# rossumur/espflix

Measured on NVIDIA H100. Metric: 352x192 MPEG-1 frames/sec (decoded YUV bit-exact vs reference), higher is better.
Workload: dtype int32/u8

## Files before the change

espflix_b200/csrc/ef_decode.cu:

```cuda
#include "ef_common.cuh"
#include "ef_coef_step.cuh"

namespace {

constexpr int kParseThreads = EF_K1A_THREADS;
constexpr int kParseCtasPerSm = EF_K1A_CTAS;
constexpr int kHdrBatch = EF_K1A_HDR_BATCH;
constexpr int kReconWarps = EF_K1B_WARPS;
constexpr int kReconCtasPerSm = EF_K1B_CTAS;

constexpr int kDenseStride = 72;
constexpr int kDenseWords = 6 * kDenseStride;
constexpr int kDenseBytes = kDenseWords * 4;
constexpr int kStageBytes = 4 * EF_TILE;
constexpr int kWarpBytes = 2 * (kDenseBytes + kStageBytes) + 16;
constexpr int kReconQzBytes = EF_K1B_DEQUANT ? 128 * 4 : 0;

struct SharedTables {
    uint16_t dct[26 * 32];
    uint16_t mba[8 * 32];
    uint16_t mv[7 * 32];
    uint16_t cbp[512];
    uint8_t ptype[64];
    uint8_t qdef[128];
    uint16_t zp[64];
    uint32_t qz[128];
};
constexpr int kTableBytes = (sizeof(SharedTables) + 15) & ~15;
constexpr int kLutBits = EF_K1A_LUT_BITS;
constexpr int kLutSize = 1 << kLutBits;
constexpr int kLutBytes = kLutBits > 0 ? 2 * kLutSize * (int)sizeof(uint2) : 0;

#if EF_K1A_ES16
constexpr int kRingStride = kParseThreads * 16;
constexpr int kRingBytes = 4 * kRingStride;
#else
constexpr int kRingStride = kParseThreads * 4;
constexpr int kRingBytes = 8 * kRingStride;
#endif
constexpr int kFlushUnroll = EF_K1A_FLUSH_UNROLL;
constexpr int kStage = EF_K1A_STAGE;
constexpr int kStageRow = EF_K1A_ES16 ? ((kStage * 4 + 16 + 15) & ~15) : (kStage + 1) * 4;
constexpr int kStageBytesA = kStage > 0 ? kParseThreads * kStageRow : 0;

struct BitReader {
    const uint32_t* words;
    uint32_t rp;
    uint32_t sring;
    uint32_t hi, lo;
#if EF_K1A_RING_AHEAD || EF_K1A_ES16
    uint32_t nx;
#endif
    int pos;

#if EF_K1A_ES16
    __device__ __forceinline__ void copy_chunk(uint32_t cidx)
    {
        asm volatile("cp.async.cg.shared.global [%0], [%1], 16;" ::"r"(sring + (cidx & 3u) * kRingStride), "l"((const uint4*)words + cidx) : "memory");
        asm volatile("cp.async.commit_group;" ::: "memory");
    }
    __device__ __forceinline__ void init(const uint8_t* blob, uint64_t byte_off)
    {
        words = (const uint32_t*)blob;
        const uint32_t w0 = (uint32_t)(byte_off >> 2);
        pos = (int)(byte_off & 3) * 8;
        asm volatile("cp.async.wait_all;" ::: "memory");
        rp = w0 + 2;
        const uint32_t c0 = (rp + 1) >> 2;
#pragma unroll
        for (int k = 0; k < 4; k++) copy_chunk(c0 + k);
        hi = __byte_perm(__ldg(words + w0), 0, 0x0123); lo = __byte_perm(__ldg(words + w0 + 1), 0, 0x0123);
        nx = __ldg(words + w0 + 2);
    }
    __device__ __forceinline__ uint32_t peek() const { return __funnelshift_l(lo, hi, pos); }
    __device__ __forceinline__ void skip(int n)
    {
// ... 32 lines not shown
    {
        pos += n;
        if (pos >= 32) {
            pos -= 32; hi = lo;
#if EF_K1A_RING_AHEAD
            lo = __byte_perm(nx, 0, 0x0123);
            asm volatile("cp.async.wait_group 5;" ::: "memory");
            asm volatile("ld.shared.u32 %0, [%1];" : "=r"(nx) : "r"(sring + ((rp + 1) & 7u) * kRingStride) : "memory");
            copy_in(rp + 7);
#else
            asm volatile("cp.async.wait_group 6;" ::: "memory");
            uint32_t raw;
            asm volatile("ld.shared.u32 %0, [%1];" : "=r"(raw) : "r"(sring + (rp & 7u) * kRingStride) : "memory");
            lo = __byte_perm(raw, 0, 0x0123);
            copy_in(rp + 7);
#endif
#if EF_K1A_PF_L2
            if ((rp & 7u) == 0) asm volatile("prefetch.global.L2 [%0];" ::"l"(words + rp + 32));
#endif
            rp++;
        }
    }
#endif
    __device__ __forceinline__ uint32_t get(int n)
    {
        uint32_t v = peek() >> (32 - n);
        skip(n);
        return v;
    }
};

struct SliceState {
    BitReader br;
    uint32_t* wptr;
    uint32_t slot_base;
    uint32_t seqi;
    const uint32_t* qzp;
    const uint32_t* qz;
    int mbw, mbh;
    int mb_x, mb_y;
    int first;
    int ptype, full_pel, r_size;
    int qscale;
    int dc_y, dc_cr, dc_cb;
    int mv_h, mv_v;
};

__device__ __forceinline__ int motion_component(uint32_t w, int& used, const uint16_t* mvtab, int m, int r_size, bool& bad)
{
    const uint32_t bits = w << used;
    int lz = __clz(bits);
    if (lz > 6) { bad = true; return m; }
    uint32_t e = mvtab[lz * 32 + ((bits << (lz + 1)) >> 27)];
    int len = e & 15;
    if (!len) { bad = true; return m; }
    int code = (int)(e >> 4) - 16;
    used += len;
    int d = code;
    if (code != 0 && r_size != 0) {
        d = ((abs(code) - 1) << r_size) + (int)((w << used) >> (32 - r_size)) + 1;
        used += r_size;
        if (code < 0) d = -d;
    }
    int scale = 1 << r_size;
    m += d;
    if (m > (scale << 4) - 1) m -= scale << 5;
    else if (m < -(scale << 4)) m += scale << 5;
// ... 7 lines not shown
    int b3 = v[2] + v[6];
    int b4 = v[5] - v[3];
    int t1 = v[1] + v[7];
    int t2 = v[3] + v[5];
    int b6 = v[1] - v[7];
    int b7 = t1 + t2;
    int m0 = kFinal ? v[0] + 128 : v[0];
    int x4 = ((b6 * 473 - b4 * 196 + 128) >> 8) - b7;
    int x0 = x4 - (((t1 - t2) * 362 + 128) >> 8);
    int x1 = m0 - b1;
    int x2 = (((v[2] - v[6]) * 362 + 128) >> 8) - b3;
    int x3 = m0 + b1;
    int y3 = x1 + x2, y4 = x3 + b3, y5 = x1 - x2, y6 = x3 - b3;
    int y7 = -x0 - ((b4 * 473 + b6 * 196 + 128) >> 8);
    v[0] = b7 + y4; v[1] = x4 + y3; v[2] = y5 - x0; v[3] = y6 - y7;
    v[4] = y6 + y7; v[5] = x0 + y5; v[6] = y3 - x4; v[7] = y4 - b7;
}

__device__ __forceinline__ uint32_t pin4(uint32_t pred, int r0, int r1, int r2, int r3)
{
#if EF_K1B_PIN16
    const uint32_t s01 = __viaddmin_s16x2_relu(__byte_perm(pred, 0, 0x4140), __byte_perm((uint32_t)r0, (uint32_t)r1, 0x6521), 0x00F800F8u);
    const uint32_t s23 = __viaddmin_s16x2_relu(__byte_perm(pred, 0, 0x4342), __byte_perm((uint32_t)r2, (uint32_t)r3, 0x6521), 0x00F800F8u);
    return __byte_perm(s01, s23, 0x6420);
#else
    const int p0 = __viaddmin_s32_relu((int)__byte_perm(pred, 0, 0x4404), r0, 0xF8FF);
    const int p1 = __viaddmin_s32_relu((int)__byte_perm(pred, 0, 0x4414), r1, 0xF8FF);
    const int p2 = __viaddmin_s32_relu((int)__byte_perm(pred, 0, 0x4424), r2, 0xF8FF);
    const int p3 = __viaddmin_s32_relu((int)__byte_perm(pred, 0, 0x4434), r3, 0xF8FF);
    return __byte_perm(__byte_perm(p0, p1, 0x0051), __byte_perm(p2, p3, 0x0051), 0x5410);
#endif
}

__device__ __forceinline__ uint32_t avg2x4(uint32_t a, uint32_t b) { return (a | b) - (((a ^ b) >> 1) & 0x7F7F7F7Fu); }

__device__ __forceinline__ uint32_t avg4x4(uint32_t a, uint32_t b, uint32_t c, uint32_t d)
{
    const uint32_t m = 0x00FF00FFu;
    uint32_t e = (a & m) + (b & m) + (c & m) + (d & m) + 0x00020002u;
    uint32_t o = ((a >> 8) & m) + ((b >> 8) & m) + ((c >> 8) & m) + ((d >> 8) & m) + 0x00020002u;
    return ((e >> 2) & m) | (((o >> 2) & m) << 8);
}

struct PredWords { uint32_t a0, a1, a2, b0, b1, b2; };

__device__ __forceinline__ uint32_t smem_u32(const void* p) { return (uint32_t)__cvta_generic_to_shared(p); }
__device__ __forceinline__ void mbar_init(uint64_t* bar, int count)
{
    asm volatile("mbarrier.init.shared::cta.b64 [%0], %1;" ::"r"(smem_u32(bar)), "r"(count));
    asm volatile("fence.mbarrier_init.release.cluster;" ::: "memory");
}
__device__ __forceinline__ void mbar_expect_tx(uint32_t sbar, uint32_t bytes)
{
    asm volatile("mbarrier.arrive.expect_tx.shared::cta.b64 _, [%0], %1;" ::"r"(sbar), "r"(bytes) : "memory");
}
__device__ __forceinline__ void bulk_tiles(uint32_t sdst, const uint8_t* gsrc, uint32_t bytes, uint32_t sbar)
{
    asm volatile("cp.async.bulk.shared::cluster.global.mbarrier::complete_tx::bytes [%0], [%1], %2, [%3];"
                 ::"r"(sdst), "l"(gsrc), "r"(bytes), "r"(sbar) : "memory");
}
__device__ __forceinline__ void mbar_wait(uint32_t sbar, uint32_t parity)
{
    uint32_t ok;
    do {
        asm volatile("{ .reg .pred p; mbarrier.try_wait.parity.shared::cta.b64 p, [%1], %2; selp.u32 %0, 1, 0, p; }"
                     : "=r"(ok) : "r"(sbar), "r"(parity) : "memory");
    } while (!ok);
}

template <bool kLuma>
__device__ __forceinline__ void pred_words_staged(const uint8_t* st, int plane, int x, int y, int tx0, int ty0, bool yh, PredWords& w)
{
    constexpr int TS = kLuma ? 16 : 8, SH = kLuma ? 4 : 3;
    const int xa = x & ~3, xi = xa & (TS - 1), yi = y & (TS - 1);
    const int o0 = ((y >> SH) - ty0) * (2 * EF_TILE) + ((xa >> SH) - tx0) * EF_TILE + (kLuma ? 0 : 256 + plane * 64) + yi * TS + xi;
    const int o1 = o0 + (xi + 4 < TS ? 4 : EF_TILE + 4 - TS);
    const int xj = (xi + 4) & (TS - 1);
    int o2 = o1 + (xj + 4 < TS ? 4 : EF_TILE + 4 - TS);
    if (((xa + 8) >> SH) - tx0 > 1) o2 = o1;
    w.a0 = *(const uint32_t*)(st + o0); w.a1 = *(const uint32_t*)(st + o1); w.a2 = *(const uint32_t*)(st + o2);
    if (yh) {
        const int d = yi == TS - 1 ? 2 * EF_TILE - (TS - 1) * TS : TS;
        w.b0 = *(const uint32_t*)(st + o0 + d); w.b1 = *(const uint32_t*)(st + o1 + d); w.b2 = *(const uint32_t*)(st + o2 + d);
    }
}

template <bool kLuma>
__device__ __forceinline__ void pred_words_clamped(const uint8_t* ref, int plane, int x, int y, bool yh, PredWords& w)
{
    constexpr int W = kLuma ? EF_W : EF_W / 2, H = kLuma ? EF_H : EF_H / 2, TS = kLuma ? 16 : 8, SH = kLuma ? 4 : 3;
    const int plane_off = kLuma ? 0 : 256 + plane * 64;
#pragma unroll
    for (int r = 0; r < 2; r++) {
        if (r == 1 && !yh) break;
        const int yy = max(0, min(H - 1, y + r));
        const int xa = max(0, min(W - 4, x & ~3)), xb = min(W - 4, xa + 4), xc = min(W - 4, xa + 8);
        const int rowbase = (yy >> SH) * EF_MBW_MAX * EF_TILE + plane_off + (yy & (TS - 1)) * TS;
        const uint32_t v0 = *(const uint32_t*)(ref + rowbase + (xa >> SH) * EF_TILE + (xa & (TS - 1)));
        const uint32_t v1 = *(const uint32_t*)(ref + rowbase + (xb >> SH) * EF_TILE + (xb & (TS - 1)));
        const uint32_t v2 = *(const uint32_t*)(ref + rowbase + (xc >> SH) * EF_TILE + (xc & (TS - 1)));
        if (r == 0) { w.a0 = v0; w.a1 = v1; w.a2 = v2; } else { w.b0 = v0; w.b1 = v1; w.b2 = v2; }
    }
}

__device__ __forceinline__ void pred_finish(const PredWords& w, int x, int xh, int yh, uint32_t& o0, uint32_t& o1)
{
    const int sh = (x & 3) * 8;
    const uint32_t p0 = __funnelshift_r(w.a0, w.a1, sh), p1 = __funnelshift_r(w.a1, w.a2, sh);
    if (xh) {
        const uint32_t q0 = __funnelshift_rc(w.a0, w.a1, sh + 8), q1 = __funnelshift_rc(w.a1, w.a2, sh + 8);
        if (yh) {
            o0 = avg4x4(p0, q0, __funnelshift_r(w.b0, w.b1, sh), __funnelshift_rc(w.b0, w.b1, sh + 8));
            o1 = avg4x4(p1, q1, __funnelshift_r(w.b1, w.b2, sh), __funnelshift_rc(w.b1, w.b2, sh + 8));
        } else {
            o0 = avg2x4(p0, q0);
            o1 = avg2x4(p1, q1);
        }
    } else if (yh) {
        o0 = avg2x4(p0, __funnelshift_r(w.b0, w.b1, sh));
        o1 = avg2x4(p1, __funnelshift_r(w.b1, w.b2, sh));
    } else {
        o0 = p0; o1 = p1;
    }
}

__device__ __forceinline__ bool parse_header(SliceState& s, const SharedTables& T, int& cbp_out, int& intra_out, uint32_t& skip_out, uint32_t& mv_out)
{
    BitReader& br = s.br;
    uint32_t bits = br.peek();
    if ((bits >> 9) == 0) return false;

    int increment = 0, used;
    uint32_t w;
    for (;;) {
        w = br.peek();
        int lz = __clz(w);
        if (lz > 7) return false;
        uint32_t e = T.mba[lz * 32 + ((w << (lz + 1)) >> 27)];
        int len = e & 15, val = (int)(e >> 4);
        if (!len) return false;
        if (val >= 34) {
            br.skip(len);
            if (val == 35) increment += 33;
            continue;
        }
        increment += val;
        used = len;
        break;
    }
    int skip_before = 0;
    if (s.first) { s.first = 0; increment = 1; }
    else if (increment > 1) { s.dc_y = s.dc_cr = s.dc_cb = 128; s.mv_h = s.mv_v = 0; skip_before = increment - 1; }
    s.mb_x += increment;
// ... 70 lines not shown
        if (delta & (1 << (dc_size - 1))) dc += delta;
        else dc += (int)((0xFFFFFFFFu << dc_size) | (uint32_t)(delta + 1));
        if (blk < 4) s.dc_y = dc; else if (blk == 4) s.dc_cr = dc; else s.dc_cb = dc;
    }
    br.skip(used + dc_size);
    return dc;
}

}

__global__ void __launch_bounds__(kParseThreads, kParseCtasPerSm)
ef_parse_kernel(const __grid_constant__ EfDev D, int pic0, int n_pics)
{
    extern __shared__ __align__(16) uint8_t smem[];
    SharedTables& T = *(SharedTables*)smem;
    const uint2* lut = (const uint2*)(smem + kTableBytes);
    {
        const uint32_t* src = (const uint32_t*)D.tables;
        uint32_t* dst = (uint32_t*)smem;
        for (int i = threadIdx.x; i < (int)(sizeof(SharedTables) / 4); i += blockDim.x) dst[i] = src[i];
        const uint4* lsrc = (const uint4*)D.tables->lut2;
        uint4* ldst = (uint4*)(smem + kTableBytes);
        for (int i = threadIdx.x; i < kLutBytes / 16; i += blockDim.x) ldst[i] = lsrc[i];
    }
    __syncthreads();
    const int lane = threadIdx.x & 31;

    uint32_t total = 0;
    for (int p = pic0; p < pic0 + n_pics; p++) total += D.pic_total[p];
    const EfWork* work = D.work + D.pic_base[pic0];
    const uint32_t n_slots = (uint32_t)D.n_streams * (EF_MBW_MAX * EF_MBH_MAX);

    SliceState s;
    s.first = 0; s.wptr = nullptr; s.slot_base = 0; s.qz = nullptr; s.mbw = 0; s.mb_x = s.mb_y = 0;
    s.br.sring = smem_u32(smem + kTableBytes + kLutBytes) + threadIdx.x * (EF_K1A_ES16 ? 16 : 4);
    const uint32_t sstage_warp = smem_u32(smem + kTableBytes + kLutBytes + kRingBytes) + (threadIdx.x & ~31u) * kStageRow;
#if EF_K1A_ES16
    const uint32_t sstage_bias = smem_u32(smem + kTableBytes + kLutBytes + kRingBytes) - (kStageRow / 16) * smem_u32(smem + kTableBytes + kLutBytes);
#define EF_SSTAGE (s.br.sring * (kStageRow / 16) + sstage_bias)
#else
    const uint32_t sstage = sstage_warp + lane * kStageRow;
#define EF_SSTAGE sstage
#endif
    bool active = false, exhausted = false, busy = false;
    uint32_t info_acc = 0, cnt = 0, skipw = 0, mvw = 0, slot = 0;
    uint32_t blk24 = 0, blkbit = 0;
    int cbp_rem = 0, n = 0, intra = 0, ctx = 0;
    auto start_block = [&]() {
        const int blk = __ffs(cbp_rem) - 1;
#if EF_K1B_DEQUANT
        blk24 = ((uint32_t)blk << 27) | ((uint32_t)s.qscale << 16);
#else
        blk24 = (uint32_t)blk << 24;
#endif
        blkbit = 0x100u << blk;
        cbp_rem &= cbp_rem - 1;
        n = 0; ctx = 1;
        if (intra) { D.mb_rec[slot].dc[blk] = parse_dc(s, blk); n = 1; ctx = 0; }
    };
    auto put_entry = [&](uint32_t ent) {
#if EF_PROBE_NOSTORE
        if (ent == 0x12345678u) s.wptr[cnt] = ent;
#else
        if (kStage > 0 && cnt < (uint32_t)kStage) asm volatile("st.shared.u32 [%0], %1;" ::"r"(EF_SSTAGE + cnt * 4), "r"(ent) : "memory");
        else s.wptr[cnt] = ent;
#endif
        cnt++;
    };
    const uint32_t first_round = gridDim.x * blockDim.x;
    bool first_fill = true;

    for (;;) {
        if (kStage > 0) {
            __syncwarp();
            const uint64_t li_mine = (uint64_t)(s.wptr - D.coef);
            if (kStage <= 32 && kHdrBatch == 32) {
                const uint32_t c_mine = (!busy && (info_acc & 1u)) ? min(cnt, (uint32_t)kStage) : 0u;
                if (__any_sync(0xFFFFFFFFu, c_mine != 0)) {
                    const uint32_t srow = sstage_warp + lane * 4;
#pragma unroll (kFlushUnroll)
                    for (int src = 0; src < 32; src++) {
                        const uint32_t c = __shfl_sync(0xFFFFFFFFu, c_mine, src);
                        const uint64_t lb = (uint64_t)__shfl_sync(0xFFFFFFFFu, (uint32_t)li_mine, src) | ((uint64_t)__shfl_sync(0xFFFFFFFFu, (uint32_t)(li_mine >> 32), src) << 32);
                        if (lane < c) {
                            uint32_t v;
                            asm volatile("ld.shared.u32 %0, [%1];" : "=r"(v) : "r"(srow + (uint32_t)src * kStageRow) : "memory");
                            D.coef[lb + lane] = v;
                        }
                    }
                }
            } else {
                unsigned owed = __ballot_sync(0xFFFFFFFFu, !busy && (info_acc & 1u) && cnt != 0);
                while (owed) {
                    const int src = __ffs(owed) - 1;
                    owed &= owed - 1;
                    const uint32_t c = min(__shfl_sync(0xFFFFFFFFu, cnt, src), (uint32_t)kStage);
                    const uint64_t lb = (uint64_t)__shfl_sync(0xFFFFFFFFu, (uint32_t)li_mine, src) | ((uint64_t)__shfl_sync(0xFFFFFFFFu, (uint32_t)(li_mine >> 32), src) << 32);
                    for (uint32_t j = lane; j < c; j += 32) {
                        uint32_t v;
                        asm volatile("ld.shared.u32 %0, [%1];" : "=r"(v) : "r"(sstage_warp + (uint32_t)src * kStageRow + j * 4) : "memory");
                        D.coef[lb + j] = v;
                    }
                }
            }
            __syncwarp();
        }
        if (!busy && (info_acc & 1u)) {
            const uint64_t li = (uint64_t)(s.wptr - D.coef);
            *(uint4*)(D.mb_rec + slot) = make_uint4(cnt | (skipw << 16), mvw, (uint32_t)li, (uint32_t)(li >> 32));
            s.wptr += cnt;
#if EF_K1B_DEQUANT
            if (s.qz) { info_acc |= 1u << 26; D.mb_rec[slot].pad[0] = s.seqi; }
#endif
            D.mb_info[slot] = info_acc | ((uint32_t)s.mbw << 20) | ((s.slot_base >> 31) << 25);
            info_acc = 0;
        }
        do {
            unsigned need = __ballot_sync(0xFFFFFFFFu, !active && !exhausted);
            if (need) {
                uint32_t base;
                if (first_fill) {
                    base = (blockIdx.x * blockDim.x + threadIdx.x) & ~31u;
                    first_fill = false;
                } else {
                    base = 0;
                    int leader = __ffs(need) - 1;
                    if (lane == leader) base = first_round + atomicAdd(D.parse_cursor, (uint32_t)__popc(need));
                    base = __shfl_sync(0xFFFFFFFFu, base, leader);
                }
                if (!active && !exhausted) {
                    uint32_t idx = base + (uint32_t)__popc(need & ((1u << lane) - 1));
                    if (idx >= total) exhausted = true;
                    else {
                        const EfWork w = work[idx];
                        const int code = w.info & 255;
                        s.ptype = (w.info >> 8) & 7; s.full_pel = (w.info >> 11) & 1; s.r_size = (w.info >> 12) & 7;
                        const EfSeq* seq = D.seq + (size_t)w.stream * (D.max_seq + 1) + (w.info >> 16);
                        s.mbw = min((int)seq->mb_width, EF_MBW_MAX);
                        s.mbh = min((int)seq->mb_height, EF_MBH_MAX);
                        s.qz = seq->custom ? (const uint32_t*)seq->qz : nullptr;
                        s.seqi = w.info >> 16;
                        s.qzp = s.qz ? s.qz : T.qz;
                        const uint64_t byte_off = D.es_off[w.stream] + w.es_off;
                        s.slot_base = (w.pic - (uint32_t)pic0) * n_slots + w.stream * (uint32_t)(EF_MBW_MAX * EF_MBH_MAX);
                        s.slot_base |= ((D.base_pics[w.stream] + w.pic + 1u) & 1u) << 31;
                        s.wptr = D.coef + 3 * byte_off;
                        s.br.init(D.es, byte_off);
                        s.mb_y = code - 2; s.mb_x = s.mbw - 1;
                        s.first = 1;
                        s.dc_y = s.dc_cr = s.dc_cb = 128; s.mv_h = s.mv_v = 0;
                        active = code >= 1 && code <= s.mbh && s.mbw > 0 && seq->valid;
                        if (active) {
                            s.qscale = (int)s.br.get(5);
                            while (s.br.get(1)) s.br.skip(8);
                        }
                    }
                }
            }
            if (active && !busy && !(info_acc & 1u)) {
                if (parse_header(s, T, cbp_rem, intra, skipw, mvw)) {
                    slot = (s.slot_base & 0x7FFFFFFFu) + (uint32_t)(s.mb_y * EF_MBW_MAX + s.mb_x);
                    info_acc = 1u | ((uint32_t)intra << 1) | ((uint32_t)cbp_rem << 2);
                    cnt = 0;
                    busy = cbp_rem != 0;
                    if (busy) start_block();
                } else active = false;
            }
        } while (__any_sync(0xFFFFFFFFu, !active && !exhausted));
        if (!__any_sync(0xFFFFFFFFu, active)) break;

#if EF_K1A_V3
        const int qoff = intra ? 0 : 64, kq = intra ? 0 : 1;
        const uint32_t* const qrow = s.qzp + qoff;
        for (;;) {
            const unsigned bmask = __ballot_sync(0xFFFFFFFFu, busy);
            if (!bmask) break;
            if (kHdrBatch < 32 && __popc(__ballot_sync(0xFFFFFFFFu, active && !busy)) >= kHdrBatch) break;
#pragma unroll
            for (int u_ = 0; u_ < EF_K1A_UNROLL; u_++)
            if (busy) {
                BitReader& br = s.br;
                const uint32_t w = br.peek();
                const EfSym sy = ef_coef_sym(w, ctx != 0, T.dct);
                ctx = 0;
                int len = sy.len;
                bool block_done = sy.kind == EF_SYM_EOB;
                if (sy.kind == EF_SYM_DERAIL) {
                    info_acc |= (blkbit << 6) | ((uint32_t)cbp_rem << 14);
                    s.mb_y = s.mbh;
                    busy = false;
                } else {
                    if (sy.kind == EF_SYM_COEF) {
                        n += sy.run;
                        if (n > 63) { info_acc |= blkbit << 6; block_done = true; }
                        else {
#if EF_K1B_DEQUANT
                            put_entry(blk24 | ((uint32_t)n << 21) | ((uint32_t)sy.lvl & 0xFFFFu));
#else
                            put_entry(ef_coef_entry(qrow[n], sy.lvl, s.qscale, kq, blk24));
#endif
                            n++;
                            if (len <= 30 && ((w << len) >> 30) == 2u) { len += 2; block_done = true; }
                        }
                    }
                    br.skip(len);
                    if (block_done) {
                        if (n == 1) info_acc |= blkbit;
                        busy = cbp_rem != 0;
                        if (busy) start_block();
                    }
                }
            }
        }
#else
        const int qoff = intra ? 0 : 64;
        const int kq = intra ? 0 : 1;
        auto qword = [&](int pos) -> uint32_t { return s.qz ? __ldg(s.qz + qoff + pos) : T.qz[qoff + pos]; };
        for (;;) {
            const unsigned bmask = __ballot_sync(0xFFFFFFFFu, busy);
            if (!bmask) break;
            if (kHdrBatch < 32 && __popc(__ballot_sync(0xFFFFFFFFu, active && !busy)) >= kHdrBatch) break;
            if (busy) {
                BitReader& br = s.br;
                const uint32_t w = br.peek();
                const EfCoefStep st = ef_coef_step(w, ctx != 0, n, lut, T.dct);
                const uint32_t fl = st.fl;
                const int len = st.len;
                ctx = 0;
                if (fl & EF_STEP_COEF1) { n += st.run1; put_entry(ef_coef_entry(qword(n), st.lvl1, s.qscale, kq, blk24)); n++; }
                if (fl & EF_STEP_COEF2) { n += st.run2; put_entry(ef_coef_entry(qword(n), st.lvl2, s.qscale, kq, blk24)); n++; }
                if (fl & 16u) {
                    info_acc |= (blkbit << 6) | ((uint32_t)cbp_rem << 14);
                    s.mb_y = s.mbh;
                    busy = false;
                } else {
                    br.skip(len);
                    if (fl & 12u) {
                        if (fl & 8u) info_acc |= blkbit << 6;
                        else if (n == 1) info_acc |= blkbit;
                        busy = cbp_rem != 0;
                        if (busy) start_block();
                    }
                }
            }
        }
#endif
    }
}

__global__ void __launch_bounds__(kReconWarps * 32, kReconCtasPerSm)
ef_recon_kernel(const __grid_constant__ EfDev D, int pic_rel)
{
    extern __shared__ __align__(16) uint8_t smem[];
    const int lane = threadIdx.x & 31, warp = threadIdx.x >> 5;
    const int hl = lane & 15, hb = lane & 16, half = lane >> 4;
    uint8_t* wbase = smem + (size_t)warp * kWarpBytes;
    int* dense = (int*)wbase + half * kDenseWords;
    uint8_t* stage = wbase + 2 * kDenseBytes + half * kStageBytes;
    uint64_t* bar = (uint64_t*)(wbase + 2 * kDenseBytes + 2 * kStageBytes) + half;
    const uint32_t sstage = smem_u32(stage), sbar = smem_u32(bar);
    uint32_t bar_phase = 0;
    if (hl == 0) mbar_init(bar, 1);
    for (int i = hl; i < kDenseWords; i += 16) dense[i] = 0;
#if EF_K1B_DEQUANT
    const uint32_t* qzs = (const uint32_t*)(smem + (size_t)kReconWarps * kWarpBytes);
    for (int i = threadIdx.x; i < 128; i += blockDim.x) ((uint32_t*)qzs)[i] = D.tables->qz[i];
    __syncthreads();
#endif
    __syncwarp();

    constexpr uint32_t kMbs = EF_MBW_MAX * EF_MBH_MAX;
    const uint32_t n_slots = (uint32_t)D.n_streams * kMbs;
    const uint32_t* infos = D.mb_info + (size_t)pic_rel * n_slots;
    const uint32_t* recs = (const uint32_t*)(D.mb_rec + (size_t)pic_rel * n_slots);

    const int ccol = hl & 7, cpb = hl >> 3;
    const int prow = hl >> 1, phalf = hl & 1;
    const int crow = hl & 7, cplane = hl >> 3;

    auto fetch = [&](uint32_t slot) -> uint32_t {
// ... 38 lines not shown
        if (hl + 32 < entries) e2 = __ldg(rl + hl + 32);

        const int mvh = (int)(int16_t)(mvw & 0xFFFF), mvv = (int)(int16_t)(mvw >> 16);
        const int tile = ef_tile_offset(mx, my);
        const int hx = mx * 32 + mvh, hy = my * 32 + mvv;
        const int cx = hx >> 1, cy = hy >> 1;
        const int X0 = hx >> 1, Y0 = hy >> 1, tx0 = X0 >> 4, ty0 = Y0 >> 4;
        const bool inside = hx >= 0 && hy >= 0 && X0 + 16 + (hx & 1) <= EF_W && Y0 + 16 + (hy & 1) <= EF_H;
        if (do_mc && inside && hl == 0) {
            const bool two_x = ((X0 + 15 + (hx & 1)) >> 4) != tx0, two_y = ((Y0 + 15 + (hy & 1)) >> 4) != ty0;
            const uint8_t* src = ref + ef_tile_offset(tx0, ty0);
            const uint32_t row_bytes = two_x ? 2 * EF_TILE : EF_TILE;
            mbar_expect_tx(sbar, row_bytes << (int)two_y);
            bulk_tiles(sstage, src, row_bytes, sbar);
            if (two_y) bulk_tiles(sstage + 2 * EF_TILE, src + EF_MBW_MAX * EF_TILE, row_bytes, sbar);
        }

        if (skip_before) {
            int sx = mx, sy = my;
            for (int k = 0; k < skip_before; k++) {
                if (--sx < 0) { sx = mbw - 1; sy--; }
                if (sy < 0) break;
                const int to = ef_tile_offset(sx, sy);
                *(uint4*)(cur + to + hl * 16) = *(const uint4*)(ref + to + hl * 16);
                *(uint2*)(cur + to + 256 + hl * 8) = *(const uint2*)(ref + to + 256 + hl * 8);
            }
        }

#if EF_K1B_DEQUANT
        const int qoff = intra_r ? 0 : 64, kq = intra_r ? 0 : 1;
        const uint32_t seqi = __shfl_sync(0xFFFFFFFFu, recw, hb + 10);
        const uint32_t* cqz = nullptr;
        if (valid && ((info >> 26) & 1u)) cqz = D.seq[(size_t)stream * (D.max_seq + 1) + min(seqi, (uint32_t)D.max_seq)].qz;
#define EF_EXPAND(ent) { const uint32_t t_ = (ent); const int eb = (t_ >> 27) & 7; if (!((abm >> eb) & 1)) { const int n_ = qoff + ((t_ >> 21) & 63); \
            const uint32_t z_ = cqz ? __ldg(cqz + n_) : qzs[n_]; dense[eb * kDenseStride + ((z_ >> 18) & 63)] = ef_dequant(z_, (int)(int16_t)(t_ & 0xFFFFu), (int)((t_ >> 16) & 31u), kq); } }
#else
#define EF_EXPAND(ent) { const uint32_t hi_ = (ent) + 0x20000u; const int eb = (hi_ >> 24) & 7; if (!((abm >> eb) & 1)) dense[eb * kDenseStride + ((hi_ >> 18) & 63)] = ((int)((ent) << 14)) >> 14; }
#endif
        if (hl < entries) EF_EXPAND(e0)
        if (hl + 16 < entries) EF_EXPAND(e1)
        if (hl + 32 < entries) EF_EXPAND(e2)
        for (int j = hl + 48; j < entries; j += 16) { const uint32_t ent = __ldg(rl + j); EF_EXPAND(ent) }
#undef EF_EXPAND
        __syncwarp();

        unsigned pass_on = 0;
#pragma unroll
        for (int p = 0; p < 3; p++) {
            if (!__any_sync(0xFFFFFFFFu, live & (3 << (2 * p)))) continue;
            pass_on |= 1u << p;
            const int bk = 2 * p + cpb;
            const int dc_col = (int)__shfl_sync(0xFFFFFFFFu, recw, hb + 4 + bk);
            int* db = dense + bk * kDenseStride + ccol;
            int v[8];
#pragma unroll
            for (int rr = 0; rr < 8; rr++) v[rr] = db[rr * 8];
            if (intra_r && ccol == 0) v[0] = (int)((uint32_t)dc_col << 8);
            idct8<false>(v);
#pragma unroll
            for (int rr = 0; rr < 8; rr++) db[rr * 8] = v[rr];
        }
        __syncwarp();

        if (do_mc && inside) { mbar_wait(sbar, bar_phase); bar_phase ^= 1; }

#pragma unroll
        for (int p = 0; p < 3; p++) {
            const bool luma = p < 2;
            const int oblk = luma ? 2 * p + phalf : 4 + cplane;
            const int orow = luma ? prow : crow;
            int w[8], dcv = 0;
#pragma unroll
            for (int i = 0; i < 8; i++) w[i] = 0;
            if (pass_on & (1u << p)) {
                const int dc_row = (int)__shfl_sync(0xFFFFFFFFu, recw, hb + 4 + oblk);
                int4* rowp = (int4*)(dense + oblk * kDenseStride + orow * 8);
                const int4 a = rowp[0], b = rowp[1];
                rowp[0] = make_int4(0, 0, 0, 0); rowp[1] = make_int4(0, 0, 0, 0);
                w[0] = a.x; w[1] = a.y; w[2] = a.z; w[3] = a.w; w[4] = b.x; w[5] = b.y; w[6] = b.z; w[7] = b.w;
                if ((live >> oblk) & 1) {
                    if (!((n1m >> oblk) & 1)) idct8<true>(w);
                    else {
                        dcv = intra_r ? dc_row : w[0] >> 8;
#pragma unroll
                        for (int i = 0; i < 8; i++) w[i] = dcv * 256;
                    }
                }
            }
            uint32_t q0 = 0, q1 = 0;
            if (do_mc) {
                PredWords pw;
                if (luma) {
                    const int lx = (hx >> 1) + phalf * 8, ly = (hy >> 1) + p * 8 + prow;
                    if (inside) pred_words_staged<true>(stage, 0, lx, ly, tx0, ty0, hy & 1, pw);
                    else pred_words_clamped<true>(ref, 0, lx, ly, hy & 1, pw);
                    pred_finish(pw, lx, hx & 1, hy & 1, q0, q1);
                } else {
                    const int kx = cx >> 1, ky = (cy >> 1) + crow;
                    if (inside) pred_words_staged<false>(stage, cplane, kx, ky, tx0, ty0, cy & 1, pw);
                    else pred_words_clamped<false>(ref, cplane, kx, ky, cy & 1, pw);
                    pred_finish(pw, kx, cx & 1, cy & 1, q0, q1);
                }
            }
            const bool coded = (cbp >> oblk) & 1, aborted = (abm >> oblk) & 1, n1 = (n1m >> oblk) & 1;
            uint32_t o0 = q0, o1 = q1;
            bool store = valid;
            if (coded && !aborted) {
                if (intra_r && n1) {
                    uint32_t d = (uint32_t)dcv; d |= d << 8; d |= d << 16;
                    o0 = o1 = d;
                } else {
                    o0 = pin4(q0, w[0], w[1], w[2], w[3]);
                    o1 = pin4(q1, w[4], w[5], w[6], w[7]);
                }
            } else if (intra_r) store = false;
            uint8_t* dst = cur + tile + (luma ? (p * 8 + prow) * 16 + phalf * 8 : 256 + cplane * 64 + crow * 8);
            if (store) *(uint2*)dst = make_uint2(o0, o1);
        }
        __syncwarp();
    }
}

size_t ef_recon_smem_bytes() { return (size_t)kReconWarps * kWarpBytes + kReconQzBytes; }
static constexpr size_t kParseSmemBytes = (size_t)kTableBytes + kLutBytes + kRingBytes + kStageBytesA;

static int g_parse_ctas = kParseCtasPerSm, g_recon_ctas = kReconCtasPerSm;

cudaError_t ef_decode_configure()
{
    cudaError_t e = cudaFuncSetAttribute(ef_recon_kernel, cudaFuncAttributeMaxDynamicSharedMemorySize, (int)ef_recon_smem_bytes());
    if (e != cudaSuccess) return e;
    e = cudaFuncSetAttribute(ef_recon_kernel, cudaFuncAttributePreferredSharedMemoryCarveout, cudaSharedmemCarveoutMaxShared);
    if (e != cudaSuccess) return e;
    int n = 0;
// ... 31 lines not shown
```

espflix_b200/csrc/ef_common.cuh:

```cuda
#pragma once
#include <cuda_runtime.h>
#include <stdint.h>

#define EF_W 352
#define EF_H 192
#define EF_STRIDE 528
#define EF_FRAME 101376
#define EF_MBW_MAX 22
#define EF_MBH_MAX 12
#define EF_TILE 384
#ifndef EF_K1A_THREADS
#define EF_K1A_THREADS 224
#endif
#ifndef EF_K1A_CTAS
#define EF_K1A_CTAS 4
#endif
#ifndef EF_K1A_PF_L2
#define EF_K1A_PF_L2 1
#endif
#ifndef EF_K1A_HDR_BATCH
#define EF_K1A_HDR_BATCH 32
#endif
#ifndef EF_K1A_V3
#define EF_K1A_V3 1
#endif
#ifndef EF_K1B_DEQUANT
#define EF_K1B_DEQUANT 0
#endif
#ifndef EF_K1A_ES16
#define EF_K1A_ES16 1
#endif
#ifndef EF_K1A_STAGE
#define EF_K1A_STAGE 32
#endif
#ifndef EF_K1A_UNROLL
#define EF_K1A_UNROLL 3
#endif
#ifndef EF_K1A_FLUSH_UNROLL
#define EF_K1A_FLUSH_UNROLL 4
#endif
#ifndef EF_PROBE_NOSTORE
#define EF_PROBE_NOSTORE 0
#endif
#ifndef EF_K1A_RING_AHEAD
#define EF_K1A_RING_AHEAD 1
#endif
#ifndef EF_K1A_LUT_BITS
#if EF_K1A_V3
#define EF_K1A_LUT_BITS 0
#else
#define EF_K1A_LUT_BITS 10
#endif
#endif
#ifndef EF_K1B_PIN16
#define EF_K1B_PIN16 1
#endif
#ifndef EF_K1B_WARPS
#define EF_K1B_WARPS 7
#endif
#ifndef EF_K1B_CTAS
#define EF_K1B_CTAS 4
#endif

struct EfTables {
    uint16_t dct[26 * 32];
    uint16_t mba[8 * 32];
    uint16_t mv[7 * 32];
    uint16_t cbp[512];
    uint8_t ptype[64];
    uint8_t qdef[128];
    uint16_t zp[64];
    uint32_t qz[128];
// ... 101 lines not shown
```

Baseline: 3.142 million.

## Streamline recon: hoist MC address math, branchless coefficient scatter, fold DC into IDCT

Motion-compensation staged-address computation is split into column/row/down parts and hoisted ahead of the barrier wait, so the per-plane work becomes pointer adds. The coefficient expansion is made branchless by sending out-of-range entries to a dummy slot. Intra DC is written into the dense buffer before the column IDCT instead of being shuffled per pass, and n1 (DC-only) blocks now go through the row IDCT with a bias correction. The 4-way byte average is replaced with a carry-save formulation. Together these cut shuffles, branches and address arithmetic in the per-row reconstruction loop, at the cost of extra IDCT work on DC-only blocks and tighter bit-exactness assumptions.

```diff
diff --git a/espflix_b200/csrc/ef_decode.cu b/espflix_b200/csrc/ef_decode.cu
--- a/espflix_b200/csrc/ef_decode.cu
+++ b/espflix_b200/csrc/ef_decode.cu
@@ -1,5 +1,6 @@
 #include "ef_common.cuh"
 #include "ef_coef_step.cuh"
+#include "ef_pixel_avg.cuh"
 
 namespace {
 
@@ -214,16 +215,6 @@
 #endif
 }
 
-__device__ __forceinline__ uint32_t avg2x4(uint32_t a, uint32_t b) { return (a | b) - (((a ^ b) >> 1) & 0x7F7F7F7Fu); }
-
-__device__ __forceinline__ uint32_t avg4x4(uint32_t a, uint32_t b, uint32_t c, uint32_t d)
-{
-    const uint32_t m = 0x00FF00FFu;
-    uint32_t e = (a & m) + (b & m) + (c & m) + (d & m) + 0x00020002u;
-    uint32_t o = ((a >> 8) & m) + ((b >> 8) & m) + ((c >> 8) & m) + ((d >> 8) & m) + 0x00020002u;
-    return ((e >> 2) & m) | (((o >> 2) & m) << 8);
-}
-
 struct PredWords { uint32_t a0, a1, a2, b0, b1, b2; };
 
 __device__ __forceinline__ uint32_t smem_u32(const void* p) { return (uint32_t)__cvta_generic_to_shared(p); }
@@ -250,21 +241,38 @@
     } while (!ok);
 }
 
+struct StagedCols { int o0, s1, s2; };
 template <bool kLuma>
-__device__ __forceinline__ void pred_words_staged(const uint8_t* st, int plane, int x, int y, int tx0, int ty0, bool yh, PredWords& w)
+__device__ __forceinline__ StagedCols staged_cols(int x, int tx0, int plane)
 {
     constexpr int TS = kLuma ? 16 : 8, SH = kLuma ? 4 : 3;
-    const int xa = x & ~3, xi = xa & (TS - 1), yi = y & (TS - 1);
-    const int o0 = ((y >> SH) - ty0) * (2 * EF_TILE) + ((xa >> SH) - tx0) * EF_TILE + (kLuma ? 0 : 256 + plane * 64) + yi * TS + xi;
-    const int o1 = o0 + (xi + 4 < TS ? 4 : EF_TILE + 4 - TS);
-    const int xj = (xi + 4) & (TS - 1);
-    int o2 = o1 + (xj + 4 < TS ? 4 : EF_TILE + 4 - TS);
-    if (((xa + 8) >> SH) - tx0 > 1) o2 = o1;
-    w.a0 = *(const uint32_t*)(st + o0); w.a1 = *(const uint32_t*)(st + o1); w.a2 = *(const uint32_t*)(st + o2);
-    if (yh) {
-        const int d = yi == TS - 1 ? 2 * EF_TILE - (TS - 1) * TS : TS;
-        w.b0 = *(const uint32_t*)(st + o0 + d); w.b1 = *(const uint32_t*)(st + o1 + d); w.b2 = *(const uint32_t*)(st + o2 + d);
-    }
+    const int xa = x & ~3, xi = xa & (TS - 1), xj = (xi + 4) & (TS - 1);
+    StagedCols c;
+    c.o0 = ((xa >> SH) - tx0) * EF_TILE + (kLuma ? 0 : 256 + plane * 64) + xi;
+    c.s1 = xi + 4 < TS ? 4 : EF_TILE + 4 - TS;
+    c.s2 = ((xa + 8) >> SH) - tx0 > 1 ? 0 : (xj + 4 < TS ? 4 : EF_TILE + 4 - TS);
+    return c;
+}
+template <bool kLuma>
+__device__ __forceinline__ int staged_row(int y, int ty0)
+{
+    constexpr int TS = kLuma ? 16 : 8, SH = kLuma ? 4 : 3;
+    return ((y >> SH) - ty0) * (2 * EF_TILE) + (y & (TS - 1)) * TS;
+}
+template <bool kLuma>
+__device__ __forceinline__ int staged_down(int y)
+{
+    constexpr int TS = kLuma ? 16 : 8;
+    return (y & (TS - 1)) == TS - 1 ? 2 * EF_TILE - (TS - 1) * TS : TS;
+}
+
+__device__ __forceinline__ void pred_words_staged(const uint8_t* st, int o, int s1, int s2, int down, bool yh, PredWords& w)
+{
+    const uint8_t* p0 = st + o;
+    const uint8_t* p1 = p0 + s1;
+    const uint8_t* p2 = p1 + s2;
+    w.a0 = *(const uint32_t*)p0; w.a1 = *(const uint32_t*)p1; w.a2 = *(const uint32_t*)p2;
+    if (yh) { w.b0 = *(const uint32_t*)(p0 + down); w.b1 = *(const uint32_t*)(p1 + down); w.b2 = *(const uint32_t*)(p2 + down); }
 }
 
 template <bool kLuma>
@@ -285,22 +293,21 @@
     }
 }
 
-__device__ __forceinline__ void pred_finish(const PredWords& w, int x, int xh, int yh, uint32_t& o0, uint32_t& o1)
-{
-    const int sh = (x & 3) * 8;
+__device__ __forceinline__ void pred_finish(const PredWords& w, int sh, bool xh, bool yh, uint32_t& o0, uint32_t& o1)
+{
     const uint32_t p0 = __funnelshift_r(w.a0, w.a1, sh), p1 = __funnelshift_r(w.a1, w.a2, sh);
     if (xh) {
         const uint32_t q0 = __funnelshift_rc(w.a0, w.a1, sh + 8), q1 = __funnelshift_rc(w.a1, w.a2, sh + 8);
         if (yh) {
-            o0 = avg4x4(p0, q0, __funnelshift_r(w.b0, w.b1, sh), __funnelshift_rc(w.b0, w.b1, sh + 8));
-            o1 = avg4x4(p1, q1, __funnelshift_r(w.b1, w.b2, sh), __funnelshift_rc(w.b1, w.b2, sh + 8));
+            o0 = ef_avg4_u8x4(p0, q0, __funnelshift_r(w.b0, w.b1, sh), __funnelshift_rc(w.b0, w.b1, sh + 8));
+            o1 = ef_avg4_u8x4(p1, q1, __funnelshift_r(w.b1, w.b2, sh), __funnelshift_rc(w.b1, w.b2, sh + 8));
         } else {
-            o0 = avg2x4(p0, q0);
-            o1 = avg2x4(p1, q1);
+            o0 = ef_avg2_u8x4(p0, q0);
+            o1 = ef_avg2_u8x4(p1, q1);
         }
     } else if (yh) {
-        o0 = avg2x4(p0, __funnelshift_r(w.b0, w.b1, sh));
-        o1 = avg2x4(p1, __funnelshift_r(w.b1, w.b2, sh));
+        o0 = ef_avg2_u8x4(p0, __funnelshift_r(w.b0, w.b1, sh));
+        o1 = ef_avg2_u8x4(p1, __funnelshift_r(w.b1, w.b2, sh));
     } else {
         o0 = p0; o1 = p1;
     }
@@ -755,35 +762,41 @@
         const uint32_t seqi = __shfl_sync(0xFFFFFFFFu, recw, hb + 10);
         const uint32_t* cqz = nullptr;
         if (valid && ((info >> 26) & 1u)) cqz = D.seq[(size_t)stream * (D.max_seq + 1) + min(seqi, (uint32_t)D.max_seq)].qz;
-#define EF_EXPAND(ent) { const uint32_t t_ = (ent); const int eb = (t_ >> 27) & 7; if (!((abm >> eb) & 1)) { const int n_ = qoff + ((t_ >> 21) & 63); \
+#define EF_EXPAND(ent, in_list) if (in_list) { const uint32_t t_ = (ent); const int eb = (t_ >> 27) & 7; if (!((abm >> eb) & 1)) { const int n_ = qoff + ((t_ >> 21) & 63); \
             const uint32_t z_ = cqz ? __ldg(cqz + n_) : qzs[n_]; dense[eb * kDenseStride + ((z_ >> 18) & 63)] = ef_dequant(z_, (int)(int16_t)(t_ & 0xFFFFu), (int)((t_ >> 16) & 31u), kq); } }
 #else
-#define EF_EXPAND(ent) { const uint32_t hi_ = (ent) + 0x20000u; const int eb = (hi_ >> 24) & 7; if (!((abm >> eb) & 1)) dense[eb * kDenseStride + ((hi_ >> 18) & 63)] = ((int)((ent) << 14)) >> 14; }
-#endif
-        if (hl < entries) EF_EXPAND(e0)
-        if (hl + 16 < entries) EF_EXPAND(e1)
-        if (hl + 32 < entries) EF_EXPAND(e2)
-        for (int j = hl + 48; j < entries; j += 16) { const uint32_t ent = __ldg(rl + j); EF_EXPAND(ent) }
+#define EF_EXPAND(ent, in_list) { const uint32_t hi_ = (ent) + 0x20000u; const int eb = (hi_ >> 24) & 7; const bool st_ = (in_list) && !((abm >> eb) & 1); \
+            dense[st_ ? eb * kDenseStride + (int)((hi_ >> 18) & 63) : 64 + ccol] = ((int)((ent) << 14)) >> 14; }
+#endif
+        EF_EXPAND(e0, hl < entries)
+        EF_EXPAND(e1, hl + 16 < entries)
+        if (hl + 32 < entries) EF_EXPAND(e2, true)
+        for (int j = hl + 48; j < entries; j += 16) { const uint32_t ent = __ldg(rl + j); EF_EXPAND(ent, true) }
 #undef EF_EXPAND
+        if (intra_r && hl >= 4 && hl < 10 && ((live >> (hl - 4)) & 1)) dense[(hl - 4) * kDenseStride] = (int)(recw << 8);
         __syncwarp();
 
-        unsigned pass_on = 0;
+        const unsigned live_w = __reduce_or_sync(0xFFFFFFFFu, (unsigned)live);
 #pragma unroll
         for (int p = 0; p < 3; p++) {
-            if (!__any_sync(0xFFFFFFFFu, live & (3 << (2 * p)))) continue;
-            pass_on |= 1u << p;
-            const int bk = 2 * p + cpb;
-            const int dc_col = (int)__shfl_sync(0xFFFFFFFFu, recw, hb + 4 + bk);
-            int* db = dense + bk * kDenseStride + ccol;
+            if (!((live_w >> (2 * p)) & 3u)) continue;
+            int* db = dense + (2 * p + cpb) * kDenseStride + ccol;
             int v[8];
 #pragma unroll
             for (int rr = 0; rr < 8; rr++) v[rr] = db[rr * 8];
-            if (intra_r && ccol == 0) v[0] = (int)((uint32_t)dc_col << 8);
             idct8<false>(v);
 #pragma unroll
             for (int rr = 0; rr < 8; rr++) db[rr * 8] = v[rr];
         }
         __syncwarp();
+
+        const bool lxh = hx & 1, lyh = hy & 1, cxh = cx & 1, cyh = cy & 1;
+        const int lsh = (hx & 6) * 4, csh = (cx & 6) * 4;
+        const StagedCols lc = staged_cols<true>(X0 + phalf * 8, tx0, 0), cc = staged_cols<false>(cx >> 1, tx0, cplane);
+        const int ly0 = Y0 + prow, cy0 = (cy >> 1) + crow;
+        const int lo0 = lc.o0 + staged_row<true>(ly0, ty0), lo1 = lc.o0 + staged_row<true>(ly0 + 8, ty0);
+        const int ldn0 = staged_down<true>(ly0), ldn1 = staged_down<true>(ly0 + 8);
+        const int co = cc.o0 + staged_row<false>(cy0, ty0), cdn = staged_down<false>(cy0);
 
         if (do_mc && inside) { mbar_wait(sbar, bar_phase); bar_phase ^= 1; }
 
@@ -793,36 +806,25 @@
             const int oblk = luma ? 2 * p + phalf : 4 + cplane;
             const int orow = luma ? prow : crow;
             int w[8], dcv = 0;
-#pragma unroll
-            for (int i = 0; i < 8; i++) w[i] = 0;
-            if (pass_on & (1u << p)) {
-                const int dc_row = (int)__shfl_sync(0xFFFFFFFFu, recw, hb + 4 + oblk);
+            if ((live_w >> (2 * p)) & 3u) {
                 int4* rowp = (int4*)(dense + oblk * kDenseStride + orow * 8);
                 const int4 a = rowp[0], b = rowp[1];
                 rowp[0] = make_int4(0, 0, 0, 0); rowp[1] = make_int4(0, 0, 0, 0);
                 w[0] = a.x; w[1] = a.y; w[2] = a.z; w[3] = a.w; w[4] = b.x; w[5] = b.y; w[6] = b.z; w[7] = b.w;
-                if ((live >> oblk) & 1) {
-                    if (!((n1m >> oblk) & 1)) idct8<true>(w);
-                    else {
-                        dcv = intra_r ? dc_row : w[0] >> 8;
-#pragma unroll
-                        for (int i = 0; i < 8; i++) w[i] = dcv * 256;
-                    }
-                }
+                if ((n1m >> oblk) & 1) { dcv = w[0] >> 8; w[0] -= 128; }
+                idct8<true>(w);
             }
             uint32_t q0 = 0, q1 = 0;
             if (do_mc) {
                 PredWords pw;
                 if (luma) {
-                    const int lx = (hx >> 1) + phalf * 8, ly = (hy >> 1) + p * 8 + prow;
-                    if (inside) pred_words_staged<true>(stage, 0, lx, ly, tx0, ty0, hy & 1, pw);
-                    else pred_words_clamped<true>(ref, 0, lx, ly, hy & 1, pw);
-                    pred_finish(pw, lx, hx & 1, hy & 1, q0, q1);
+                    if (inside) pred_words_staged(stage, p == 0 ? lo0 : lo1, lc.s1, lc.s2, p == 0 ? ldn0 : ldn1, lyh, pw);
+                    else pred_words_clamped<true>(ref, 0, X0 + phalf * 8, ly0 + p * 8, lyh, pw);
+                    pred_finish(pw, lsh, lxh, lyh, q0, q1);
                 } else {
-                    const int kx = cx >> 1, ky = (cy >> 1) + crow;
-                    if (inside) pred_words_staged<false>(stage, cplane, kx, ky, tx0, ty0, cy & 1, pw);
-                    else pred_words_clamped<false>(ref, cplane, kx, ky, cy & 1, pw);
-                    pred_finish(pw, kx, cx & 1, cy & 1, q0, q1);
+                    if (inside) pred_words_staged(stage, co, cc.s1, cc.s2, cdn, cyh, pw);
+                    else pred_words_clamped<false>(ref, cplane, cx >> 1, cy0, cyh, pw);
+                    pred_finish(pw, csh, cxh, cyh, q0, q1);
                 }
             }
             const bool coded = (cbp >> oblk) & 1, aborted = (abm >> oblk) & 1, n1 = (n1m >> oblk) & 1;
diff --git a/espflix_b200/csrc/ef_pixel_avg.cuh b/espflix_b200/csrc/ef_pixel_avg.cuh
--- /dev/null
+++ b/espflix_b200/csrc/ef_pixel_avg.cuh
@@ -0,0 +1,22 @@
+#pragma once
+#include <stdint.h>
+#if !defined(__CUDACC__) && !defined(__host__)
+#define __host__
+#define __device__
+#define __forceinline__ inline
+#endif
+
+static __host__ __device__ __forceinline__ uint32_t ef_avg2_u8x4(uint32_t a, uint32_t b)
+{
+    return (a | b) - (((a ^ b) >> 1) & 0x7F7F7F7Fu);
+}
+
+static __host__ __device__ __forceinline__ uint32_t ef_avg4_u8x4(uint32_t a, uint32_t b, uint32_t c, uint32_t d)
+{
+    const uint32_t k = 0x02020202u;
+    const uint32_t s1 = a ^ b ^ c, c1 = (a & b) | (c & (a | b));
+    const uint32_t s2 = s1 ^ d ^ k, c2 = (s1 & d) | (k & (s1 | d));
+    const uint32_t h = (s2 >> 1) & 0x7F7F7F7Fu;
+    const uint32_t s3 = c1 ^ c2 ^ h, c3 = (c1 & c2) | (h & (c1 | c2));
+    return c3 + ((s3 >> 1) & 0x7F7F7F7Fu);
+}
```

Result: faster. 3.187 million, median of 6 (+1.5%).

## Stage coefficient entries in a shared ring and flush cooperatively by slice

Applied to the files above, without the earlier changes.

Replaces the per-macroblock staging (first 32 entries in shared memory, overflow written directly to global) with a 32-entry circular shared ring per thread. Each slice's coefficient list is contiguous, and the warp flushes pending entries cooperatively with coalesced stores whenever a thread's backlog nears ring capacity or a thread needs a new slice. The per-MB flush at every loop top goes away, and the header-batch threshold drops from 32 to 24 so finished lanes can fetch new headers earlier. The cost is extra warp-wide ballots each symbol-loop pass and more frequent, smaller flushes.

```diff
diff --git a/espflix_b200/csrc/ef_common.cuh b/espflix_b200/csrc/ef_common.cuh
--- a/espflix_b200/csrc/ef_common.cuh
+++ b/espflix_b200/csrc/ef_common.cuh
@@ -19,7 +19,7 @@
 #define EF_K1A_PF_L2 1
 #endif
 #ifndef EF_K1A_HDR_BATCH
-#define EF_K1A_HDR_BATCH 32
+#define EF_K1A_HDR_BATCH 24
 #endif
 #ifndef EF_K1A_V3
 #define EF_K1A_V3 1
@@ -30,14 +30,8 @@
 #ifndef EF_K1A_ES16
 #define EF_K1A_ES16 1
 #endif
-#ifndef EF_K1A_STAGE
-#define EF_K1A_STAGE 32
-#endif
 #ifndef EF_K1A_UNROLL
 #define EF_K1A_UNROLL 3
-#endif
-#ifndef EF_K1A_FLUSH_UNROLL
-#define EF_K1A_FLUSH_UNROLL 4
 #endif
 #ifndef EF_PROBE_NOSTORE
 #define EF_PROBE_NOSTORE 0
diff --git a/espflix_b200/csrc/ef_decode.cu b/espflix_b200/csrc/ef_decode.cu
--- a/espflix_b200/csrc/ef_decode.cu
+++ b/espflix_b200/csrc/ef_decode.cu
@@ -38,10 +38,11 @@
 constexpr int kRingStride = kParseThreads * 4;
 constexpr int kRingBytes = 8 * kRingStride;
 #endif
-constexpr int kFlushUnroll = EF_K1A_FLUSH_UNROLL;
-constexpr int kStage = EF_K1A_STAGE;
+constexpr int kStage = 32;
+constexpr int kStageHigh = kStage - (EF_K1A_V3 ? EF_K1A_UNROLL : 2);
+static_assert(kStageHigh > 0, "a pass of the symbol loop must fit in the staging ring");
 constexpr int kStageRow = EF_K1A_ES16 ? ((kStage * 4 + 16 + 15) & ~15) : (kStage + 1) * 4;
-constexpr int kStageBytesA = kStage > 0 ? kParseThreads * kStageRow : 0;
+constexpr int kStageBytesA = kParseThreads * kStageRow;
 
 struct BitReader {
     const uint32_t* words;
@@ -140,7 +141,7 @@
 
 struct SliceState {
     BitReader br;
-    uint32_t* wptr;
+    uint32_t* list;
     uint32_t slot_base;
     uint32_t seqi;
     const uint32_t* qzp;
@@ -437,7 +438,7 @@
     const uint32_t n_slots = (uint32_t)D.n_streams * (EF_MBW_MAX * EF_MBH_MAX);
 
     SliceState s;
-    s.first = 0; s.wptr = nullptr; s.slot_base = 0; s.qz = nullptr; s.mbw = 0; s.mb_x = s.mb_y = 0;
+    s.first = 0; s.list = D.coef; s.slot_base = 0; s.qz = nullptr; s.mbw = 0; s.mb_x = s.mb_y = 0;
     s.br.sring = smem_u32(smem + kTableBytes + kLutBytes) + threadIdx.x * (EF_K1A_ES16 ? 16 : 4);
     const uint32_t sstage_warp = smem_u32(smem + kTableBytes + kLutBytes + kRingBytes) + (threadIdx.x & ~31u) * kStageRow;
 #if EF_K1A_ES16
@@ -448,7 +449,8 @@
 #define EF_SSTAGE sstage
 #endif
     bool active = false, exhausted = false, busy = false;
-    uint32_t info_acc = 0, cnt = 0, skipw = 0, mvw = 0, slot = 0;
+    uint32_t tot = 0, done = 0;
+    uint32_t info_acc = 0, mb0 = 0, skipw = 0, mvw = 0, slot = 0;
     uint32_t blk24 = 0, blkbit = 0;
     int cbp_rem = 0, n = 0, intra = 0, ctx = 0;
     auto start_block = [&]() {
@@ -464,56 +466,38 @@
         if (intra) { D.mb_rec[slot].dc[blk] = parse_dc(s, blk); n = 1; ctx = 0; }
     };
     auto put_entry = [&](uint32_t ent) {
-#if EF_PROBE_NOSTORE
-        if (ent == 0x12345678u) s.wptr[cnt] = ent;
-#else
-        if (kStage > 0 && cnt < (uint32_t)kStage) asm volatile("st.shared.u32 [%0], %1;" ::"r"(EF_SSTAGE + cnt * 4), "r"(ent) : "memory");
-        else s.wptr[cnt] = ent;
-#endif
-        cnt++;
+        asm volatile("st.shared.u32 [%0], %1;" ::"r"(EF_SSTAGE + (tot % kStage) * 4), "r"(ent) : "memory");
+        tot++;
+    };
+    auto flush = [&]() {
+        __syncwarp();
+#if !EF_PROBE_NOSTORE
+        const uint32_t pend = tot - done;
+        const uint64_t dst = (uint64_t)(s.list + done);
+        const uint32_t key = pend | (done << 8);
+        unsigned owed = __ballot_sync(0xFFFFFFFFu, pend != 0);
+        while (owed) {
+            const int src = __ffs(owed) - 1;
+            owed &= owed - 1;
+            const uint32_t k = __shfl_sync(0xFFFFFFFFu, key, src);
+            uint32_t* const d = (uint32_t*)((uint64_t)__shfl_sync(0xFFFFFFFFu, (uint32_t)dst, src) | ((uint64_t)__shfl_sync(0xFFFFFFFFu, (uint32_t)(dst >> 32), src) << 32));
+            if ((uint32_t)lane < (k & 255u)) {
+                uint32_t v;
+                asm volatile("ld.shared.u32 %0, [%1];" : "=r"(v) : "r"(sstage_warp + (uint32_t)src * kStageRow + (((k >> 8) + lane) % kStage) * 4) : "memory");
+                d[lane] = v;
+            }
+        }
+#endif
+        __syncwarp();
+        done = tot;
     };
     const uint32_t first_round = gridDim.x * blockDim.x;
     bool first_fill = true;
 
     for (;;) {
-        if (kStage > 0) {
-            __syncwarp();
-            const uint64_t li_mine = (uint64_t)(s.wptr - D.coef);
-            if (kStage <= 32 && kHdrBatch == 32) {
-                const uint32_t c_mine = (!busy && (info_acc & 1u)) ? min(cnt, (uint32_t)kStage) : 0u;
-                if (__any_sync(0xFFFFFFFFu, c_mine != 0)) {
-                    const uint32_t srow = sstage_warp + lane * 4;
-#pragma unroll (kFlushUnroll)
-                    for (int src = 0; src < 32; src++) {
-                        const uint32_t c = __shfl_sync(0xFFFFFFFFu, c_mine, src);
-                        const uint64_t lb = (uint64_t)__shfl_sync(0xFFFFFFFFu, (uint32_t)li_mine, src) | ((uint64_t)__shfl_sync(0xFFFFFFFFu, (uint32_t)(li_mine >> 32), src) << 32);
-                        if (lane < c) {
-                            uint32_t v;
-                            asm volatile("ld.shared.u32 %0, [%1];" : "=r"(v) : "r"(srow + (uint32_t)src * kStageRow) : "memory");
-                            D.coef[lb + lane] = v;
-                        }
-                    }
-                }
-            } else {
-                unsigned owed = __ballot_sync(0xFFFFFFFFu, !busy && (info_acc & 1u) && cnt != 0);
-                while (owed) {
-                    const int src = __ffs(owed) - 1;
-                    owed &= owed - 1;
-                    const uint32_t c = min(__shfl_sync(0xFFFFFFFFu, cnt, src), (uint32_t)kStage);
-                    const uint64_t lb = (uint64_t)__shfl_sync(0xFFFFFFFFu, (uint32_t)li_mine, src) | ((uint64_t)__shfl_sync(0xFFFFFFFFu, (uint32_t)(li_mine >> 32), src) << 32);
-                    for (uint32_t j = lane; j < c; j += 32) {
-                        uint32_t v;
-                        asm volatile("ld.shared.u32 %0, [%1];" : "=r"(v) : "r"(sstage_warp + (uint32_t)src * kStageRow + j * 4) : "memory");
-                        D.coef[lb + j] = v;
-                    }
-                }
-            }
-            __syncwarp();
-        }
         if (!busy && (info_acc & 1u)) {
-            const uint64_t li = (uint64_t)(s.wptr - D.coef);
-            *(uint4*)(D.mb_rec + slot) = make_uint4(cnt | (skipw << 16), mvw, (uint32_t)li, (uint32_t)(li >> 32));
-            s.wptr += cnt;
+            const uint64_t li = (uint64_t)(s.list - D.coef) + mb0;
+            *(uint4*)(D.mb_rec + slot) = make_uint4((tot - mb0) | (skipw << 16), mvw, (uint32_t)li, (uint32_t)(li >> 32));
 #if EF_K1B_DEQUANT
             if (s.qz) { info_acc |= 1u << 26; D.mb_rec[slot].pad[0] = s.seqi; }
 #endif
@@ -521,6 +505,7 @@
             info_acc = 0;
         }
         do {
+            if (__any_sync(0xFFFFFFFFu, !active && tot != done)) flush();
             unsigned need = __ballot_sync(0xFFFFFFFFu, !active && !exhausted);
             if (need) {
                 uint32_t base;
@@ -549,7 +534,8 @@
                         const uint64_t byte_off = D.es_off[w.stream] + w.es_off;
                         s.slot_base = (w.pic - (uint32_t)pic0) * n_slots + w.stream * (uint32_t)(EF_MBW_MAX * EF_MBH_MAX);
                         s.slot_base |= ((D.base_pics[w.stream] + w.pic + 1u) & 1u) << 31;
-                        s.wptr = D.coef + 3 * byte_off;
+                        s.list = D.coef + 3 * byte_off;
+                        tot = done = 0;
                         s.br.init(D.es, byte_off);
                         s.mb_y = code - 2; s.mb_x = s.mbw - 1;
                         s.first = 1;
@@ -566,21 +552,26 @@
                 if (parse_header(s, T, cbp_rem, intra, skipw, mvw)) {
                     slot = (s.slot_base & 0x7FFFFFFFu) + (uint32_t)(s.mb_y * EF_MBW_MAX + s.mb_x);
                     info_acc = 1u | ((uint32_t)intra << 1) | ((uint32_t)cbp_rem << 2);
-                    cnt = 0;
+                    mb0 = tot;
                     busy = cbp_rem != 0;
                     if (busy) start_block();
                 } else active = false;
             }
         } while (__any_sync(0xFFFFFFFFu, !active && !exhausted));
-        if (!__any_sync(0xFFFFFFFFu, active)) break;
-
+        const unsigned amask = __ballot_sync(0xFFFFFFFFu, active);
+        if (!amask) break;
+
+        const int qoff = intra ? 0 : 64, kq = intra ? 0 : 1;
 #if EF_K1A_V3
-        const int qoff = intra ? 0 : 64, kq = intra ? 0 : 1;
         const uint32_t* const qrow = s.qzp + qoff;
+#else
+        auto qword = [&](int pos) -> uint32_t { return s.qz ? __ldg(s.qz + qoff + pos) : T.qz[qoff + pos]; };
+#endif
         for (;;) {
             const unsigned bmask = __ballot_sync(0xFFFFFFFFu, busy);
-            if (!bmask) break;
-            if (kHdrBatch < 32 && __popc(__ballot_sync(0xFFFFFFFFu, active && !busy)) >= kHdrBatch) break;
+            if (!bmask || __popc(amask & ~bmask) >= kHdrBatch) break;
+            if (__any_sync(0xFFFFFFFFu, tot - done > (uint32_t)kStageHigh)) flush();
+#if EF_K1A_V3
 #pragma unroll
             for (int u_ = 0; u_ < EF_K1A_UNROLL; u_++)
             if (busy) {
@@ -616,15 +607,7 @@
                     }
                 }
             }
-        }
-#else
-        const int qoff = intra ? 0 : 64;
-        const int kq = intra ? 0 : 1;
-        auto qword = [&](int pos) -> uint32_t { return s.qz ? __ldg(s.qz + qoff + pos) : T.qz[qoff + pos]; };
-        for (;;) {
-            const unsigned bmask = __ballot_sync(0xFFFFFFFFu, busy);
-            if (!bmask) break;
-            if (kHdrBatch < 32 && __popc(__ballot_sync(0xFFFFFFFFu, active && !busy)) >= kHdrBatch) break;
+#else
             if (busy) {
                 BitReader& br = s.br;
                 const uint32_t w = br.peek();
@@ -648,9 +631,10 @@
                     }
                 }
             }
-        }
-#endif
-    }
+#endif
+        }
+    }
+#undef EF_SSTAGE
 }
 
 __global__ void __launch_bounds__(kReconWarps * 32, kReconCtasPerSm)
```

Measured after the change: 2.865 million before, 2.976 million after, median of 6. 1.04x the previous value.
